# UBCMOCCA/mocca_envs

Measured on AMD Instinct MI355X. Metric: env-steps/sec, Walker3DCustomEnv-v0 @ 4096 envs, 1/2/4/8 MI355X, higher is better.
Workload: dtype f32; 1 GPU; Walker3DCustomEnv-v0, 4096 envs/GPU, flat ground, U(-1,1) action tape, auto-reset; max_rows=48, max_contacts=12, envs_per_gpu=4096, parallelism=independent env shards x1, no collective, preroll_steps=5896

## Files before the change

### mocca_envs_amd/csrc/mocca_device.h

```cpp
#pragma once

#include <hip/hip_runtime.h>
#include <stdint.h>

#include "mocca_model.h"
#include "mocca_philox.h"
#include "topo_walker3d.h"
#include "topo_cassie.h"
#include "topo_walker2d.h"
#include "topo_crab2d.h"
#include "topo_laikago.h"

#define DI __device__ __forceinline__

#ifndef MOCCA_NS
#define MOCCA_NS mocca
#endif
#ifndef MOCCA_MAXR
#define MOCCA_MAXR 48
#endif
#ifndef MOCCA_COMPACT
#define MOCCA_COMPACT 0
#endif

// ... 872 lines not shown
DI float hf_height_at(const float* hf, int rows, int cols, float sc, float x, float y) {
  const float ox = (float)rows / sc * 0.5f, oy = (float)cols / sc * 0.5f;
  int ix = (int)((x + ox) * sc), iy = (int)((y + oy) * sc);
  ix = ix < 0 ? 0 : (ix > cols - 1 ? cols - 1 : ix);
  iy = iy < 0 ? 0 : (iy > rows - 1 ? rows - 1 : iy);
  return hf[iy * cols + ix];
}

DI float clamp01(float x) { return x < 0.0f ? 0.0f : (x > 1.0f ? 1.0f : x); }
DI void seg_seg(const float* p1, const float* q1, const float* p2, const float* q2, float* c1, float* c2) {
  float d1[3], d2[3], r[3];
#pragma unroll
  for (int k = 0; k < 3; ++k) { d1[k] = q1[k] - p1[k]; d2[k] = q2[k] - p2[k]; r[k] = p1[k] - p2[k]; }
  const float a = dot3(d1, d1), e = dot3(d2, d2), f = dot3(d2, r), EPS = 1e-12f;
  float s, t;
  if (a <= EPS && e <= EPS) { s = t = 0; }
  else if (a <= EPS) { s = 0; t = clamp01(f * rcp(e)); }
  else {
    const float c = dot3(d1, r), ia = rcp(a);
    if (e <= EPS) { t = 0; s = clamp01(-c * ia); }
    else {
      const float b = dot3(d1, d2), den = a * e - b * b;
      s = den > EPS ? clamp01((b * f - c * e) * rcp(den)) : 0.0f;
      t = (b * s + f) * rcp(e);
      if (t < 0) { t = 0; s = clamp01(-c * ia); }
      else if (t > 1) { t = 1; s = clamp01((b - c) * ia); }
    }
  }
#pragma unroll
  for (int k = 0; k < 3; ++k) { c1[k] = p1[k] + d1[k] * s; c2[k] = p2[k] + d2[k] * t; }
}

template <class T>
DI void geom_points(ModelP M, float* L, int lane) {
  static_assert(6 * T::NG <= GP_FLOATS || (T::NPAIR == 0 && !COMPACT), "geom points would overlap the contact records read by the self-collision pass");
  if (lane < 2 * T::NG) {
    const f4_t t = *(CF4P)(M->gp_tab[lane]);
    const int b = __float_as_int(t.w);
    const float pl[3] = {t.x, t.y, t.z};
#pragma unroll
    for (int i = 0; i < 3; ++i) {
      const float4 fr = *reinterpret_cast<const float4*>(L + L_RT + 12 * b + 4 * i);
      L[L_GP + 3 * lane + i] = fr.x * pl[0] + fr.y * pl[1] + fr.z * pl[2] + fr.w;
    }
  }
}

DI void stage_planks(ModelP M, float* L, int lane, const float* ter) {
  if (lane < M->n_planks) {
    const int row = (int)ter[120 + lane];
    const float* ti = ter + 6 * row;
    float Rb[9];
    euler_to_mat(ti[4], ti[5], ti[3], Rb);
    const float cz = M->plank_com_z, dz = -M->plank_half[2] - cz;
#pragma unroll
    for (int i = 0; i < 9; ++i) L[L_PLANK + 12 * lane + i] = Rb[i];
    L[L_PLANK + 12 * lane + 9] = ti[0] + Rb[2] * dz;
    L[L_PLANK + 12 * lane + 10] = ti[1] + Rb[5] * dz;
    L[L_PLANK + 12 * lane + 11] = ti[2] + Rb[8] * dz + cz;
  }
  wsync();
}

struct HeightFieldArgs { const float* data; int rows, cols; float scale; };
struct ContactFlags { int touch0, touch1, target0, target1, touch2, touch3, body_touch, target2, target3; };
DI int cover_targets(int cover, int nsi, int n_planks, int f) { return (cover >> (4 * f + nsi % n_planks)) & 1; }

template <class T, int TASK>
DI ContactFlags collide(ModelP M, float* L, int lane, const float* ter, int next_step_index,
                        int* nc_out, int32_t* dbg, int* nc_wanted, const HeightFieldArgs hfa, int* cover_out = nullptr) {
  STAMP_BEGIN;
  const float mreach = unif(M->contact_margin);
  ContactFlags fl = {0, 0, 0, 0, 0, 0, 0, 0, 0};
  const int maxc = uni(M->max_contacts);
  bool active = false;
  float n[3] = {0, 0, 1}, P[3] = {0, 0, 0}, gap = 1e30f, mu = 0, erp = M->erp, cfm = 0;
  int body = -1, slot = lane, cover_k = -1 , gfoot = -1, gtorso = 0;
  unsigned bmask = 0u;
  if (lane < T::NSLOT) {
    const f4_t st = *(CF4P)(M->slot_tab[lane]);
    const int ids = __float_as_int(st.z);
    const int g = (ids >> 8) & 0xFF, e = (ids >> 16) & 1;
    bmask = __float_as_uint(st.w);
    if ((ids >> 25) & 1) {
      gfoot = ((ids >> 26) & 7) - 1;
      gtorso = (ids >> 29) & 1;
      float C[3], Cw[3];
      const float rad = st.x, gfric = st.y;
#pragma unroll
      for (int i = 0; i < 3; ++i) { C[i] = L[L_GP + 3 * (2 * g + e) + i]; Cw[i] = C[i] + L[L_BASE + i]; }
      body = ids & 0xFF;
      if (TASK == MOCCA_TASK_WALKER3D_PLANNER) {
        gap = sphere_heightfield(hfa.data, hfa.rows, hfa.cols, hfa.scale, Cw, rad, rad + mreach, 1 + ((ids >> 30) & 3), n);
        mu = M->plank_friction * gfric;
        const float kk = M->plank_stiffness, cc = M->plank_damping, dt = M->dt;
        const float ikc = rcp(dt * kk + cc);
        erp = dt * kk * ikc;
        cfm = ikc * rcp(dt);
      } else if (TASK != MOCCA_TASK_WALKER3D_STEPPER) {
        gap = Cw[2] - rad;
        mu = M->ground_friction * gfric;
      } else {
        const float h[3] = {M->plank_half[0], M->plank_half[1], M->plank_half[2]};
        const int n_planks = M->n_planks;
        const bool cyl = M->plank_shape == MOCCA_PLANK_CYLINDER;
#pragma unroll 1
        for (int k = 0; k < n_planks; ++k) {
          float Rb[9], bc[3], nn[3];
#pragma unroll
          for (int i = 0; i < 9; ++i) Rb[i] = L[L_PLANK + 12 * k + i];
#pragma unroll
          for (int i = 0; i < 3; ++i) bc[i] = L[L_PLANK + 12 * k + 9 + i];
          float lb[3];
// ... 67 lines not shown
      fl.target1 = cover_targets(cover, next_step_index, npl, 1);
      if constexpr (T::NFEET > 2) { fl.target2 = cover_targets(cover, next_step_index, npl, 2); fl.target3 = cover_targets(cover, next_step_index, npl, 3); }
      if (cover_out) *cover_out = cover;
    }
    if (TASK == MOCCA_TASK_WALKER3D_PLANNER) fl.body_touch = __ballot(active && gtorso) != 0ull;
  }
  int nc = __popcll(am);
  const int n_terrain = nc;
  int n_self = 0;
  unsigned long long kept = am;
  if (nc > maxc) {
    int deeper = 0;
    for (unsigned long long mm = am; mm; mm &= mm - 1) {
      const int l = __builtin_ctzll(mm);
      const float gl = readlane(gap, l);
      deeper += (gl < gap || (gl == gap && l < lane)) ? 1 : 0;
    }
    kept = __ballot(active && deeper < maxc);
  }
  {
    const int idx = lane_rank(kept);
    if (active && ((kept >> lane) & 1ull)) {
      float* ct = L + L_CT + 16 * idx;
      ct[C_BA] = __int_as_float(body); ct[C_BB] = __int_as_float(-1); ct[C_SLOT] = __int_as_float(slot);
#pragma unroll
      for (int i = 0; i < 3; ++i) { ct[C_P + i] = P[i]; ct[C_N + i] = n[i]; }
      ct[C_DEPTH] = -gap; ct[C_MU] = mu; ct[C_ERP] = erp; ct[C_CFM] = cfm;
      ct[C_MA] = __uint_as_float(bmask); ct[C_MB] = __uint_as_float(0u);
    }
  }
  if (nc > maxc) nc = maxc;
  STAMP(13);
  const int npairs = uni(M->n_pairs);
  unsigned short* cand = reinterpret_cast<unsigned short*>(L + L_CAND);
  static_assert(2 * ((COMPACT ? L_ABA_END : L_TOTAL) - L_CAND) >= MOCCA_MAX_PAIRS, "candidate list must hold every pair");
  int ncand = 0;
#pragma unroll 1
  for (int base = 0; base < npairs; base += 64) {
    const int k = base + lane;
    bool near = false;
    if (k < npairs) {
#ifdef MOCCA_ABL_PAIRLOAD
      f4_t pt;
      pt.x = __int_as_float((k % T::NG) | (((k * 7 + 3) % T::NG) << 5) | (24 << 20)); pt.y = 0.05f; pt.z = 0.05f; pt.w = 0.04f;
#else
      const f4_t pt = *(CF4P)(M->pair_tab[k]);
#endif
      const int ids = __float_as_int(pt.x);
      const int ga = ids & 31, gb = (ids >> 5) & 31;
      float dm[3];
#pragma unroll
      for (int i = 0; i < 3; ++i)
        dm[i] = (L[L_GP + 6 * ga + i] + L[L_GP + 6 * ga + 3 + i]) - (L[L_GP + 6 * gb + i] + L[L_GP + 6 * gb + 3 + i]);
      const float reach = 2.0f * (pt.w + (float)((ids >> 20) & 0xFF) * (1.0f / 8192.0f));
      near = dot3(dm, dm) < reach * reach;
    }
    const unsigned long long nm = __ballot(near);
    if (near) cand[ncand + lane_rank(nm)] = (unsigned short)k;
    ncand += __popcll(nm);
  }
  ncand = uni(ncand);
#ifdef MOCCA_ABL_NOPASS2
  ncand = 0;
#endif
  wsync();
#pragma unroll 1
  for (int base = 0; base < ncand; base += 64) {
    bool hit = false;
    float nn[3] = {0, 0, 0}, PP[3] = {0, 0, 0}, g2 = 0, mu2 = 0;
    int ba = -1, bb = -1;
    if (base + lane < ncand) {
      const int k = cand[base + lane];
      const f4_t pt = *(CF4P)(M->pair_tab[k]);
      const int ids = __float_as_int(pt.x);
      const int ga = ids & 31, gb = (ids >> 5) & 31;
      float a1[3], a2[3], b1[3], b2[3];
#pragma unroll
      for (int i = 0; i < 3; ++i) {
        a1[i] = L[L_GP + 6 * ga + i]; a2[i] = L[L_GP + 6 * ga + 3 + i];
// ... 194 lines not shown
#pragma unroll 1
  for (int j = nnc - 1; j >= 0; --j) {
    const float as = Acol[MAXR * j] * invdiag;
    const float nl_ = __builtin_amdgcn_fmed3f(y, lo0, 1e30f);
    const float dl = readlane(nl_ - lam, j);
    lam = lane == j ? nl_ : lam;
    y = fmaf(-as, dl, y);
  }
}
template <int PGS_REG_ROWS, int RR>
DI void pgs_fixed_rows_from(const float* Acol, const float* ar, int start, int r_fr, float& y, float& lam, float invdiag, float lo0) {
  if constexpr (RR < MAXR) {
    if (RR >= r_fr) return;
    if (RR >= start) pgs_visit<RR>(RR < PGS_REG_ROWS ? ar[RR < PGS_REG_ROWS ? RR : 0] : Acol[MAXR * RR] * invdiag, y, lam, lo0);
    pgs_fixed_rows_from<PGS_REG_ROWS, RR + 1>(Acol, ar, start, r_fr, y, lam, invdiag, lo0);
  }
}

DI void set_issue_priority(int nr, int prio) {
  if (nr > ((prio >> 12) & 63)) __builtin_amdgcn_s_setprio(3);
  else if (nr > ((prio >> 6) & 63)) __builtin_amdgcn_s_setprio(2);
  else if (nr > (prio & 63)) __builtin_amdgcn_s_setprio(1);
  else __builtin_amdgcn_s_setprio(0);
}
#ifndef MOCCA_PACE_ROWUNIT
#define MOCCA_PACE_ROWUNIT 2
#endif
#ifndef MOCCA_PACE_SHIFT
#define MOCCA_PACE_SHIFT 4
#endif
constexpr int PACE_TICK_SHIFT = 6;
enum : int { L_T0 = L_BASE + 13, L_PACE = L_BASE + 14, L_KEEPWARM = L_BASE + 15  };
constexpr unsigned PACE_CNT_BITS = 24, PACE_WINDOW = 128;
DI void pace_start(const StepArgs& a, float* L, int lane, int pace) {
  if (lane == 0) {
    int p16 = pace >> PACE_TICK_SHIFT;
    if (pace < 0) {
      const unsigned long long v = __hip_atomic_load(a.pace_acc, __ATOMIC_RELAXED, __HIP_MEMORY_SCOPE_AGENT);
      const unsigned cnt = (unsigned)v & ((1u << PACE_CNT_BITS) - 1u);
      p16 = cnt > 0u ? (int)((float)(v >> PACE_CNT_BITS) / (float)cnt * (float)(-pace) * 0.0625f) : 0;
    }
    L[L_PACE] = __int_as_float(p16);
    if (pace != 0) L[L_T0] = __uint_as_float((unsigned)__builtin_amdgcn_s_memtime());
  }
}
DI void pace_finish(const StepArgs& a, const float* L, int lane, int pace) {
  if (pace < 0 && lane == 0 && (blockIdx.x % 61u) == 0u) {
    const unsigned el = ((unsigned)__builtin_amdgcn_s_memtime() - __float_as_uint(L[L_T0])) >> PACE_TICK_SHIFT;
    const unsigned long long old = atomicAdd(a.pace_acc, ((unsigned long long)el << PACE_CNT_BITS) | 1ull);
    if (((unsigned)old & ((1u << PACE_CNT_BITS) - 1u)) + 1u == PACE_WINDOW) {
      const unsigned long long sum = (old >> PACE_CNT_BITS) + el;
      atomicAdd(a.pace_acc, 0ull - (((sum >> 1) << PACE_CNT_BITS) | (unsigned long long)(PACE_WINDOW / 2)));
    }
  }
}
DI bool pace_on(const float* L) { return uni(__float_as_int(L[L_PACE])) > 0; }
DI void pace_checkpoint(const float* L, int done, int total) {
  const unsigned p16 = (unsigned)uni(__float_as_int(L[L_PACE]));
  if (p16 == 0u) return;
  const unsigned el = (unsigned)__builtin_amdgcn_s_memtime() - (unsigned)uni(__float_as_int(L[L_T0]));
  const unsigned lhs = (el >> PACE_TICK_SHIFT) * (unsigned)total, r = p16 * (unsigned)done;
  if (lhs > r + (r >> MOCCA_PACE_SHIFT)) __builtin_amdgcn_s_setprio(3);
  else if (lhs > r) __builtin_amdgcn_s_setprio(2);
  else if (lhs > r - (r >> MOCCA_PACE_SHIFT)) __builtin_amdgcn_s_setprio(1);
  else __builtin_amdgcn_s_setprio(0);
}
DI void dbg_fold_step(int32_t* dbg, int lane) {
  if (dbg && lane == 0) {
    unsigned long long h = ((unsigned long long)(unsigned)dbg[17] << 32) | (unsigned)dbg[16];
#pragma unroll 1
    for (int w = 0; w < 12; ++w) h = (h ^ (unsigned long long)(unsigned)dbg[w]) * 0x9E3779B97F4A7C15ull;
    dbg[16] = (int32_t)(unsigned)h; dbg[17] = (int32_t)(unsigned)(h >> 32); dbg[18] += 1;
  }
}
template <class T>
DI void solve_constraints(ModelP M, float* L, int lane, int nc_found, int nc_wanted, unsigned long long ppk, int32_t* dbg, const float* Afac, int prio, int& rows_out) {
  const bool keep_warm = uni(__float_as_int(L[L_KEEPWARM])) != 0;
  STAMP_BEGIN;
  const float dt = unif(M->dt), idt = rcp(dt);
  const int maxr = uni(M->max_rows);
  int nl;
  {
    bool act = false;
    if (lane < 2 * T::NJ) {
      const int b = 1 + (lane >> 1), side = lane & 1;
      const float q = L[L_Q + b];
      const float gap = side == 0 ? q - M->jlo[b] : M->jhi[b] - q;
      const float vel = (side == 0 ? 1.0f : -1.0f) * L[L_NU + 5 + b];
      act = M->limit_at_violation ? !(gap > 0.0f) : gap + dt * vel < M->limit_slack;
    }
    const unsigned long long lm = __ballot(act);
    const int rk = lane_rank(lm);
    if (act && rk < maxr) reinterpret_cast<int*>(L)[L_ROWD + rk] = lane;
    nl = uni(__popcll(lm));
    if (dbg && lane == 0) {
      dbg[5] = (int32_t)(unsigned)lm; dbg[6] = (int32_t)(unsigned)(lm >> 32);
      const int nfix = 3 * T::NCLOS + ((T::NCLOS > 0 && M->planar) ? 3 : 0), mc = M->max_contacts;
      const int wanted = nl + nfix + 3 * nc_wanted;
      dbg[12] += nc_wanted > mc ? 1 : 0;
      dbg[13] += nl + nfix + 3 * (nc_wanted < mc ? nc_wanted : mc) > maxr ? 1 : 0;
      dbg[14] += 1;
      if (wanted > dbg[15]) dbg[15] = wanted;
    }
    if (nl > maxr) nl = maxr;
  }
  constexpr int NCL = 3 * T::NCLOS;
  const int NFIX = NCL + ((T::NCLOS > 0 && uni(M->planar)) ? 3 : 0);
  int nc = uni(nc_found);
  if (nc > (maxr - nl - NFIX) / 3) nc = (maxr - nl - NFIX) / 3;
  if (nc < 0) nc = 0;
  const int nr = nl + NFIX + 3 * nc;
  if (dbg && lane == 0) { dbg[0] = nr; dbg[1] = nl; dbg[2] = nc; }
  if (!pace_on(L)) set_issue_priority(nr, prio);
  rows_out = nr;
  wsync();
  STAMP(16);
  if (nr == 0) {
    if (dbg && lane == 0) { dbg[8] = 0; dbg[9] = 0; dbg[10] = 0; dbg[11] = 0; }
    if (keep_warm && lane < T::NSLOT) L[L_WARM + lane] = 0.0f;
    wsync();
    return;
  }
  const int r = lane;
  const int r_fr = nl + NFIX + nc;
  const int row_gap = MAXR - nr;
  const bool is_fric = r >= MAXR - 2 * nc && r < MAXR;
  const bool has_row = r < r_fr || is_fric;
  const int ci = is_fric ? (MAXR - 1 - r) >> 1 : r - nl - NFIX;
  int kind = -1, ba = 0, bb = -1, jl = -1, slot = -1;
  float F[6] = {0, 0, 0, 0, 0, 0}, sgn = 0, bias = 0, cfm = 0, lam = 0, mu = 0;
  float F2[6] = {0, 0, 0, 0, 0, 0};
  if (r < nl) {
    const int c = reinterpret_cast<int*>(L)[L_ROWD + r];
    const int b = 1 + (c >> 1), side = c & 1;
    const float q = L[L_Q + b];
    const float gap = side == 0 ? q - M->jlo[b] : M->jhi[b] - q;
    kind = 0; jl = b; ba = b; sgn = side == 0 ? 1.0f : -1.0f;
    bias = gap < 0 ? M->erp_noncontact * (-gap) * idt : -gap * idt;
  } else if (T::NCLOS > 0 && r < nl + NCL) {
    const int c = (r - nl) / 3, ax = (r - nl) % 3;
    ba = M->cl_body_a[c]; bb = M->cl_body_b[c];
    kind = 3;
    float Pa[3], Pb[3], Ra[9], Rb[9], la[3], lb[3];
#pragma unroll
    for (int x = 0; x < 9; ++x) { Ra[x] = L[L_RT + 12 * ba + 4 * (x / 3) + x % 3]; Rb[x] = L[L_RT + 12 * bb + 4 * (x / 3) + x % 3]; }
#pragma unroll
    for (int x = 0; x < 3; ++x) { la[x] = M->cl_point_a[c][x]; lb[x] = M->cl_point_b[c][x]; }
    matvec3(Ra, la, Pa); matvec3(Rb, lb, Pb);
#pragma unroll
    for (int x = 0; x < 3; ++x) { Pa[x] += L[L_RT + 12 * ba + 4 * x + 3]; Pb[x] += L[L_RT + 12 * bb + 4 * x + 3]; }
    float dir[3] = {ax == 0 ? 1.0f : 0.0f, ax == 1 ? 1.0f : 0.0f, ax == 2 ? 1.0f : 0.0f}, pn[3];
    cross3(Pa, dir, pn);
#pragma unroll
    for (int x = 0; x < 3; ++x) { F[x] = pn[x]; F[3 + x] = dir[x]; }
    cross3(Pb, dir, pn);
#pragma unroll
    for (int x = 0; x < 3; ++x) { F2[x] = pn[x]; F2[3 + x] = dir[x]; }
    const float e = ax == 0 ? Pb[0] - Pa[0] : (ax == 1 ? Pb[1] - Pa[1] : Pb[2] - Pa[2]);
    bias = M->erp_noncontact * e * idt;
  } else if (T::NCLOS > 0 && r < nl + NFIX) {
    const int k = r - nl - NCL;
    const int comp = k == 0 ? 0 : (k == 1 ? 2 : 4);
    kind = 3; ba = 0; bb = -1;
#pragma unroll
    for (int x = 0; x < 6; ++x) F[x] = x == comp ? 1.0f : 0.0f;
    const float err = k == 0 ? L[L_RT + 9]  : (k == 1 ? -L[L_RT + 1]  : L[L_BASE + 1] - M->init_pos[1]);
    bias = -M->erp_noncontact * err * idt;
  } else if (has_row) {
    const float* ct = L + L_CT + 16 * ci;
    float n[3] = {ct[C_N], ct[C_N + 1], ct[C_N + 2]}, P[3] = {ct[C_P], ct[C_P + 1], ct[C_P + 2]}, dir[3];
    ba = __float_as_int(ct[C_BA]); bb = __float_as_int(ct[C_BB]);
    if (!is_fric) {
      kind = 1;
      dir[0] = n[0]; dir[1] = n[1]; dir[2] = n[2];
      const float depth = ct[C_DEPTH] - unif(M->linear_slop);
      bias = depth > 0 ? ct[C_ERP] * depth * idt : depth * idt;
      cfm = ct[C_CFM];
      slot = __float_as_int(ct[C_SLOT]);
      const float wsf = unif(M->warmstart);
      lam = (wsf != 0.0f && slot >= 0) ? wsf * L[L_WARM + slot] : 0.0f;
    } else {
      kind = 2;
      float t1[3], t2[3];
      plane_space(n, t1, t2);
      const bool second = (r & 1) != 0;
#pragma unroll
      for (int x = 0; x < 3; ++x) dir[x] = second ? t2[x] : t1[x];
      mu = ct[C_MU];
    }
    float pn[3];
    cross3(P, dir, pn);
#pragma unroll
    for (int x = 0; x < 3; ++x) { F[x] = pn[x]; F[3 + x] = dir[x]; F2[x] = pn[x]; F2[3 + x] = dir[x]; }
  }
  STAMP(17);
  unsigned ma = 0u, mb = 0u;
  if (kind == 1 || kind == 2) {
    const float* ct = L + L_CT + 16 * ci;
    ma = __float_as_uint(ct[C_MA]); mb = __float_as_uint(ct[C_MB]);
  } else if (kind >= 0) {
    ma = M->anc_mask[ba];
    mb = (kind == 3 && bb >= 0) ? M->anc_mask[bb] : 0u;
  }
  const float sa = kind >= 1 ? 1.0f : 0.0f, sb = (kind >= 1 && bb >= 0) ? 1.0f : 0.0f;

  STAMP(5);
  float X[T::ND];
  float w = 0;
  const int dense = has_row ? (r < r_fr ? r : r - row_gap) : MAXR;
  float* Jrow = L + L_J + 28 * dense;
  float pa[6] = {0, 0, 0, 0, 0, 0}, pb[6] = {0, 0, 0, 0, 0, 0};
#ifdef MOCCA_NO_TWO_PATHS
  const bool two_paths = false;
#else
  const bool two_paths = T::NCLOS > 0 || __ballot(kind >= 1 && bb >= 0) != 0ull;
#endif
  STAMP(18);
  const unsigned long long pka = ((unsigned long long)(unsigned)__shfl((int)(unsigned)(ppk >> 32), ba, 64) << 32) |
                                 (unsigned long long)(unsigned)__shfl((int)(unsigned)ppk, ba, 64);
  {
    float4* jz = reinterpret_cast<float4*>(Jrow);
#pragma unroll
    for (int i = 1; i < 7; ++i) jz[i] = make_float4(0.0f, 0.0f, 0.0f, 0.0f);
  }
  float pu[T::MAXD], pub[T::MAXD];
#pragma unroll
  for (int k = T::MAXD - 1; k >= 0; --k) {
    const int j = (int)((pka >> (5 * k)) & 31ull);
    const bool valid = j != 0;
    const int jj = j;
    float S[6], U[6];
#pragma unroll
    for (int i = 0; i < 6; ++i) { S[i] = L[L_SV + SVS * jj + i]; U[i] = L[L_SV + SVS * jj + SV_V + i]; }
    float jb = dot6(S, F);
    if (jj == jl) jb = sgn;
// ... 248 lines not shown
    float ax[3], jr[9], Rq[9], Tl[9];
#pragma unroll
    for (int i = 0; i < 3; ++i) ax[i] = M->jaxis[j][i];
#pragma unroll
    for (int i = 0; i < 9; ++i) jr[i] = M->jrot[j][i];
    Rq[0] = cq + t * ax[0] * ax[0];          Rq[1] = t * ax[0] * ax[1] - s * ax[2];   Rq[2] = t * ax[0] * ax[2] + s * ax[1];
    Rq[3] = t * ax[0] * ax[1] + s * ax[2];   Rq[4] = cq + t * ax[1] * ax[1];          Rq[5] = t * ax[1] * ax[2] - s * ax[0];
    Rq[6] = t * ax[0] * ax[2] - s * ax[1];   Rq[7] = t * ax[1] * ax[2] + s * ax[0];   Rq[8] = cq + t * ax[2] * ax[2];
    matmul3(jr, Rq, Tl);
    float4* rec = reinterpret_cast<float4*>(L + L_SV + SVS * j);
    rec[0] = make_float4(Tl[0], Tl[1], Tl[2], Tl[3]);
    rec[1] = make_float4(Tl[4], Tl[5], Tl[6], Tl[7]);
    rec[2] = make_float4(Tl[8], M->jpos[j][0], M->jpos[j][1], M->jpos[j][2]);
    rec[3] = make_float4(ax[0], ax[1], ax[2], L[L_QD + j]);
  }
  wsync();
}

template <class T, int TASK>
DI ContactFlags substep(ModelP M, float* L, int lane, const float* ter, int next_step_index,
                        unsigned long long ppk, int32_t* dbg, int prio, int& rows_out,
                        const HeightFieldArgs hfa = HeightFieldArgs{nullptr, 0, 0, 0.0f}, int sidx = 0, int nsub = 1, int* cover_out = nullptr) {
  const int per0 = 64 + MOCCA_PACE_ROWUNIT * rows_out, done0 = sidx * per0, total = nsub * per0;
  STAMP(30);
  stage_joints<T>(M, L, lane);
  STAMP(29);
  int nc = 0, nc_wanted = 0;
  float Afac[21] = {0, 0, 0, 0, 0, 0, 0, 0, 0, 0, 0, 0, 0, 0, 0, 0, 0, 0, 0, 0, 0};
  ContactFlags fl = {0, 0, 0, 0, 0, 0, 0, 0, 0};
  if constexpr (COMPACT) {
    static_assert(!COMPACT || T::NCLOS == 0, "closure rows read the body frames after the ABA: not in the compact layout");
    int wl = lane;
    asm volatile("" : "+v"(wl));
    walk_phase1<T>(L, wl, ppk);
    wsync();
    STAMP(0);
    geom_points<T>(M, L, lane);
    wsync();
    STAMP(15);
#ifndef MOCCA_SKIP_COLLIDE
    fl = collide<T, TASK>(M, L, lane, ter, next_step_index, &nc, dbg, &nc_wanted, hfa, cover_out);
#endif
    wsync();
    const int wb = wl < T::NB ? wl : 0;
    WalkConsts wk;
    walk_consts<true>(M, wb, wk);
    walk_phase2<T, true>(M, L, wl, wb, ppk, wk);
    wsync();
  } else {
    walk_kinematics<T, true>(M, L, lane, ppk);
    wsync();
    STAMP(0);
    geom_points<T>(M, L, lane);
    wsync();
    STAMP(15);
#ifndef MOCCA_SKIP_COLLIDE
    fl = collide<T, TASK>(M, L, lane, ter, next_step_index, &nc, dbg, &nc_wanted, hfa, cover_out);
#endif
  }
  STAMP(1);
  pace_checkpoint(L, done0 + 20, total);
#ifndef MOCCA_SKIP_ABA
  aba_passes<T>(M, L, lane, ppk, Afac);
#endif
  STAMP(2);
  pace_checkpoint(L, done0 + 36, total);
#ifndef MOCCA_SKIP_SOLVE
  solve_constraints<T>(M, L, lane, nc, nc_wanted, ppk, dbg, Afac, prio, rows_out);
#endif
  if (dbg) { __builtin_amdgcn_s_waitcnt(0); dbg_fold_step(dbg, lane); }
  STAMP(3);
#ifdef MOCCA_DUMMY_VALU
  {
    float x = (float)lane;
#ifdef MOCCA_DUMMY_ILP
    float y = x + 1.0f, z = x + 2.0f, u = x + 3.0f;
#pragma unroll 1
    for (int i = 0; i < MOCCA_DUMMY_VALU; ++i) { x = fmaf(x, 1.0001f, 0.5f); y = fmaf(y, 0.9999f, -0.5f); z = fmaf(z, 1.0001f, 0.5f); u = fmaf(u, 0.9999f, -0.5f); }
    asm volatile("" :: "v"(y), "v"(z), "v"(u));
#else
#pragma unroll 1
    for (int i = 0; i < MOCCA_DUMMY_VALU; ++i) { x = fmaf(x, 1.0001f, 0.5f); x = fmaf(x, 0.9999f, -0.5f); x = fmaf(x, 1.0001f, 0.5f); x = fmaf(x, 0.9999f, -0.5f); }
#endif
    asm volatile("" :: "v"(x));
  }
#endif
  integrate<T>(M, L, lane);
  STAMP(4);
  pace_checkpoint(L, (sidx + 1) * (64 + MOCCA_PACE_ROWUNIT * rows_out), nsub * (64 + MOCCA_PACE_ROWUNIT * rows_out));
  return fl;
// ... 429 lines not shown
  if (mode != MOCCA_CASSIE_PLAIN) {
    const float u = draw_u<INJECT>(a, env, t.episode, t.draw);
    t.draw += 1;
    int is = (int)(u * 10000.0f);
    is = is > 9999 ? 9999 : is;
    t.istep = M->cassie_rsi ? is : 0;
    frame = traj_frame(a, M, t.istep, &phase);
  }
  if (lane >= 1 && lane < T::NB) { L[L_Q + lane] = M->init_q[lane]; L[L_QD + lane] = 0.0f; }
  if (lane < MOCCA_MAX_CTRL) L[L_JVEL + lane] = 0.0f;
  wsync();
  if (mode != MOCCA_CASSIE_PLAIN) {
    const float* fr = a.traj + (size_t)frame * MOCCA_TRAJ_STRIDE;
    if (lane < M->n_ordered) {
      const int b = M->ordered_body[lane];
      L[L_Q + b] = fr[lane]; L[L_QD + b] = fr[14 + lane]; L[L_JVEL + lane] = fr[14 + lane];
    }
    if (lane < 4) { L[L_Q + M->rod_body[lane]] = fr[28 + lane]; L[L_QD + M->rod_body[lane]] = 0.0f; }
  }
  t.initz = reset_base_pose<T>(M, L, lane);
  const CassieState cs = cassie_state(M, L, lane, t.initz);
  cassie_observe(M, L, lane, cs, t.initz, lane < MOCCA_MAX_CTRL ? L[L_JVEL + lane] : 0.0f, phase, obs);
  t.linpot = cassie_potential(M, L);
}

template <class T, int TASK, bool INJECT>
DI void reset_task(const StepArgs& a, ModelP M, float* L, float* ter, uint32_t* tk, int env, int lane, TaskRegs& t, float* obs) {
  if constexpr (TASK == MOCCA_TASK_CASSIE) {
    cassie_reset_env<T, INJECT>(a, M, L, env, lane, t, obs);
    if (lane < MOCCA_MAX_CTRL) tk[MOCCA_TW_JVEL + lane] = __float_as_uint(L[L_JVEL + lane]);
  } else reset_env<T, TASK, INJECT>(a, M, L, ter, env, lane, t, obs);
}

DI void load_dyn(const float* st, float* L, int lane, int nj, int nslots, bool warm = true) {
  if (lane < 13) L[L_BASE + lane] = st[lane];
  if (lane < nj) { L[L_Q + 1 + lane] = st[13 + lane]; L[L_QD + 1 + lane] = st[13 + nj + lane]; }
  if (warm) { if (lane < nslots) L[L_WARM + lane] = st[13 + 2 * nj + lane]; }
  else if (lane < MOCCA_MAX_SLOTS) L[L_WARM + lane] = 0.0f;
}
DI void store_dyn(float* st, const float* L, int lane, int nj, int nslots, bool warm = true) {
  if (lane < 13) st[lane] = L[L_BASE + lane];
  if (lane < nj) { st[13 + lane] = L[L_Q + 1 + lane]; st[13 + nj + lane] = L[L_QD + 1 + lane]; }
  if (warm && lane < nslots) st[13 + 2 * nj + lane] = L[L_WARM + lane];
}

}
```

### mocca_envs_amd/csrc/mocca_kernels.h

```cpp
#pragma once
#include <hip/hip_runtime.h>

#include "mocca.h"
#include "mocca_device.h"

namespace MOCCA_NS {

#ifndef MOCCA_WAVES_PER_EU
#define MOCCA_WAVES_PER_EU 4
#endif

DI void flush_obs(const float* L, float* dst, int lane, int obs_dim) {
#pragma unroll 1
  for (int k = lane; k < obs_dim; k += 64) dst[k] = L[L_OBS + k];
}
DI void keep_terminal_obs(const StepArgs& a, const float* L, int env, int lane) {
  wsync();
  if (a.final_obs) flush_obs(L, a.final_obs + (size_t)env * a.obs_dim, lane, a.obs_dim);
  wsync();
}

template <class T>
DI void keep_robot_state(const StepArgs& a, const float* L, int env, int lane) {
  static_assert(ROBOT_OBS<T> <= 64 && ROBOT_OBS<T> <= ROBOT_STATE_STRIDE, "one store per lane");
// ... 179 lines not shown
template <class T>
DI StepResult cassie_step(const StepArgs& __restrict__ a, ModelP M, float* L, uint32_t* tk, int lane, unsigned long long ppk, TaskRegs& __restrict__ t,
                          float* obs) {
  t.istep += M->n_llc;
  float jv = 0.0f;
  if (lane < M->n_ordered) {
    jv = (L[L_Q + M->ordered_body[lane]] - L[L_Q0 + lane]) / M->control_dt;
    tk[MOCCA_TW_JVEL + lane] = __float_as_uint(jv);
  }
  stage_joints<T>(M, L, lane);
  walk_kinematics<T, false>(M, L, lane, ppk);
  wsync();
  t.t += 1;
  const CassieState cs = cassie_state(M, L, lane, t.initz);
  const float old = t.linpot;
  t.linpot = cassie_potential(M, L);
  const float alive = cs.height > M->alive_height ? 2.0f : -1.0f;
  if (!cs.finite || alive < 0.0f) t.done = 1;
  float rew = alive + (t.linpot - old);
  float phase = 0.0f;
  if (M->cassie_mode != MOCCA_CASSIE_PLAIN) {
    const int f1 = traj_frame(a, M, t.istep, &phase);
    rew = cassie_mocap_reward(a, M, L, lane, cs, jv, f1);
  }
  cassie_observe(M, L, lane, cs, t.initz, jv, phase, obs);
  return {rew, 0};
}

template <class T, int TASK, bool INJECT = false>
__global__ __launch_bounds__(64, MOCCA_WAVES_PER_EU) void mocca_step_kernel(StepArgs a) {
  __shared__ float L[L_TOTAL];
  const int lane = threadIdx.x;
  if ((int)blockIdx.x >= a.n_envs) return;
  const int env = a.order ? uni(a.order[blockIdx.x]) : (int)blockIdx.x;
  ModelP M = (ModelP)a.model;
  float* st = a.dyn + (size_t)env * DYN_STRIDE;
  uint32_t* tk = a.task + (size_t)env * MOCCA_TASK_WORDS;
  float* ter = TASK == MOCCA_TASK_WALKER3D_STEPPER ? a.terrain + (size_t)env * TERRAIN_STRIDE : nullptr;
  float* obs_out = a.obs + (size_t)env * a.obs_dim;
  float* obs = L + L_OBS;
  int32_t* dbg = a.dbg ? a.dbg + (size_t)env * MOCCA_DEBUG_WORDS : nullptr;

  const bool warm_ld = INJECT || uni(__float_as_int(M->warmstart)) != 0, warm_st = warm_ld || a.persist_warm != 0;
  if (dbg && lane == 0) { dbg[16] = 0; dbg[17] = 0; dbg[18] = 0; }
  load_dyn(st, L, lane, T::NJ, T::NSLOT, warm_ld);
  pace_start(a, L, lane, INJECT ? 0 : a.pace);
  if (lane == 0) L[L_KEEPWARM] = __int_as_float(warm_st ? 1 : 0);
  const unsigned long long ppk = T::path_packed(lane < T::NB ? lane : 0);
  ContactFlags fl = {0, 0, 0, 0, 0, 0, 0, 0, 0};
  int cover = 0;
  if constexpr (TASK == MOCCA_TASK_CASSIE) {
    const int no = M->n_ordered, nctl = M->n_ctrl, mode = M->cassie_mode;
    float target = 0.0f;
    if (lane < nctl) {
      float base = M->ctrl_base[lane];
      if (mode != MOCCA_CASSIE_PLAIN) {
        const int f0 = traj_frame(a, M, (int)tk[MOCCA_TW_ISTEP]);
        base = (lane < nctl - 2 && M->residual_control) ? a.traj[(size_t)f0 * MOCCA_TRAJ_STRIDE + M->ctrl_oidx[lane]] : 0.0f;
      }
      target = base + (lane < nctl - 2 ? a.act[(size_t)env * (nctl - 2) + lane] : 0.0f);
    }
    if (lane < no) {
      L[L_JVEL + lane] = __uint_as_float(tk[MOCCA_TW_JVEL + lane]);
      L[L_Q0 + lane] = L[L_Q + M->ordered_body[lane]];
    }
    if (lane < MOCCA_MAX_BODIES) L[L_TAU + lane] = 0.0f;
    if (lane == 0) { L[L_Q] = 0.0f; L[L_QD] = 0.0f; }
    wsync();
    const int nllc = INJECT ? 0 : M->n_llc;
    int last_rows = uni((int)tk[MOCCA_TW_LAST_ROWS]);
    if (!INJECT && a.pace == 0) set_issue_priority(last_rows, a.prio);
#pragma unroll 1
    for (int it = 0; it < nllc; ++it) {
      ModelP Ms = M;
      int ln = lane;
      unsigned long long pk = ppk;
      asm volatile("" : "+s"(Ms), "+v"(ln), "+v"(pk));
      if (ln < no) {
        const float al = Ms->jvel_alpha;
        L[L_JVEL + ln] = (1.0f - al) * L[L_JVEL + ln] + al * L[L_QD + Ms->ordered_body[ln]];
      }
      wsync();
      if (ln < nctl) {
        const int b = Ms->ctrl_body[ln];
        const float perr = target - L[L_Q + b];
        float verr = -L[L_JVEL + Ms->ctrl_oidx[ln]];
        verr = verr < -5.0f ? -5.0f : (verr > 5.0f ? 5.0f : verr);
        const float tq = Ms->ctrl_kp[ln] * perr + Ms->ctrl_kd[ln] * verr, lim = Ms->torque_limit[b];
        L[L_TAU + b] = tq < -lim ? -lim : (tq > lim ? lim : tq);
      }
      wsync();
      substep<T, TASK>(Ms, L, ln, nullptr, 0, pk, dbg, a.prio, last_rows, HeightFieldArgs{nullptr, 0, 0, 0.0f}, it, nllc);
    }
    if (!INJECT && lane == 0) tk[MOCCA_TW_LAST_ROWS] = (uint32_t)last_rows;
  } else {
    {
      const float applied_gain = __uint_as_float(tk[MOCCA_TW_APPLIED_GAIN]);
      if (lane < T::NJ) {
        const float act_raw = a.act[(size_t)env * T::NJ + lane];
        const float c = act_raw < -1.0f ? -1.0f : (act_raw > 1.0f ? 1.0f : act_raw);
        L[L_TAU + 1 + lane] = M->gain[lane + 1] * applied_gain * c;
      }
    }
    if (lane == 0) { L[L_TAU] = 0.0f; L[L_Q] = 0.0f; L[L_QD] = 0.0f; }
    wsync();

    STAMP(28);
    if constexpr (TASK == MOCCA_TASK_WALKER3D_STEPPER) stage_planks(M, L, lane, ter);
    const int nsub = INJECT ? 0 : M->n_substeps;
    const int nsi0 = TASK == MOCCA_TASK_WALKER3D_STEPPER ? (int)tk[MOCCA_TW_NEXT_STEP_INDEX] : 0;
    int last_rows = uni((int)tk[MOCCA_TW_LAST_ROWS]);
    if (!INJECT && a.pace == 0) set_issue_priority(last_rows, a.prio);
#pragma unroll 1
    for (int s = 0; s < nsub; ++s) {
      ModelP Ms = M;
      int ln = lane;
      unsigned long long pk = ppk;
      asm volatile("" : "+s"(Ms), "+v"(ln), "+v"(pk));
      fl = substep<T, TASK>(Ms, L, ln, ter, nsi0, pk, dbg, a.prio, last_rows, HeightFieldArgs{a.hf, a.hf_rows, a.hf_cols, a.hf_scale}, s, nsub, &cover);
    }
    if constexpr (INJECT) {
      const int32_t* tc = a.inj_touch + (size_t)env * T::NFEET;
      fl.touch0 = tc[0] != 0; fl.touch1 = tc[1] != 0;
      if constexpr (T::NFEET > 2) { fl.touch2 = tc[2] != 0; fl.touch3 = tc[3] != 0; }
      if (a.inj_target) {
        const int32_t* tg = a.inj_target + (size_t)env * T::NFEET;
        const int npl = TASK == MOCCA_TASK_WALKER3D_STEPPER ? M->n_planks : 1;
#pragma unroll
        for (int f = 0; f < T::NFEET; ++f)
          if (tg[f] == 1 || tg[f] == 2) cover |= 1 << (4 * f + (nsi0 + tg[f] - 1) % npl);
        fl.target0 = tg[0] == 1; fl.target1 = tg[1] == 1;
        if constexpr (T::NFEET > 2) { fl.target2 = tg[2] == 1; fl.target3 = tg[3] == 1; }
      }
      if (a.inj_body) fl.body_touch = a.inj_body[env] != 0;
    }
    if (!INJECT && lane == 0) tk[MOCCA_TW_LAST_ROWS] = (uint32_t)last_rows;
    STAMP(27);
  }
  TaskRegs t = load_task<T, TASK>(tk);
  const float ep_ret0 = a.ep_ret ? a.ep_ret[env] : 0.0f;
  StepResult r;
  if constexpr (TASK == MOCCA_TASK_CASSIE) r = cassie_step<T>(a, M, L, tk, lane, ppk, t, obs);
  else {
    const float act_raw = lane < T::NJ ? a.act[(size_t)env * T::NJ + lane] : 0.0f;
    {
      int lo = lane;
      asm volatile("" : "+v"(lo));
      stage_joints<T>(M, L, lo);
      walk_kinematics<T, false>(M, L, lo, ppk);
    }
    wsync();
    t.t += 1;
// ... 121 lines not shown
```

Baseline: 41.13 million env-steps/s.

## Issue global loads early and pin them in registers across kernel phases

```diff
diff --git a/mocca_envs_amd/csrc/mocca_device.h b/mocca_envs_amd/csrc/mocca_device.h
--- a/mocca_envs_amd/csrc/mocca_device.h
+++ b/mocca_envs_amd/csrc/mocca_device.h
@@ -928,10 +928,12 @@
 }
 
 template <class T>
-DI void geom_points(ModelP M, float* L, int lane) {
+DI f4_t geom_request(ModelP M, int lane) { return *(CF4P)(M->gp_tab[lane < 2 * T::NG ? lane : 0]); }
+template <class T>
+DI void geom_points(float* L, int lane, f4_t t) {
   static_assert(6 * T::NG <= GP_FLOATS || (T::NPAIR == 0 && !COMPACT), "geom points would overlap the contact records read by the self-collision pass");
+  asm volatile("" : "+v"(t));
   if (lane < 2 * T::NG) {
-    const f4_t t = *(CF4P)(M->gp_tab[lane]);
     const int b = __float_as_int(t.w);
     const float pl[3] = {t.x, t.y, t.z};
 #pragma unroll
@@ -958,13 +960,15 @@
   wsync();
 }
 
+template <class T>
+DI f4_t slot_request(ModelP M, int lane) { return *(CF4P)(M->slot_tab[lane < T::NSLOT ? lane : 0]); }
 struct HeightFieldArgs { const float* data; int rows, cols; float scale; };
 struct ContactFlags { int touch0, touch1, target0, target1, touch2, touch3, body_touch, target2, target3; };
 DI int cover_targets(int cover, int nsi, int n_planks, int f) { return (cover >> (4 * f + nsi % n_planks)) & 1; }
 
 template <class T, int TASK>
 DI ContactFlags collide(ModelP M, float* L, int lane, const float* ter, int next_step_index,
-                        int* nc_out, int32_t* dbg, int* nc_wanted, const HeightFieldArgs hfa, int* cover_out = nullptr) {
+                        int* nc_out, int32_t* dbg, int* nc_wanted, const HeightFieldArgs hfa, f4_t slot_rec, int* cover_out = nullptr) {
   STAMP_BEGIN;
   const float mreach = unif(M->contact_margin);
   ContactFlags fl = {0, 0, 0, 0, 0, 0, 0, 0, 0};
@@ -973,8 +977,9 @@
   float n[3] = {0, 0, 1}, P[3] = {0, 0, 0}, gap = 1e30f, mu = 0, erp = M->erp, cfm = 0;
   int body = -1, slot = lane, cover_k = -1 , gfoot = -1, gtorso = 0;
   unsigned bmask = 0u;
+  asm volatile("" : "+v"(slot_rec));
   if (lane < T::NSLOT) {
-    const f4_t st = *(CF4P)(M->slot_tab[lane]);
+    const f4_t st = slot_rec;
     const int ids = __float_as_int(st.z);
     const int g = (ids >> 8) & 0xFF, e = (ids >> 16) & 1;
     bmask = __float_as_uint(st.w);
@@ -1108,6 +1113,8 @@
   if (nc > maxc) nc = maxc;
   STAMP(13);
   const int npairs = uni(M->n_pairs);
+  f4_t pt_next = {0.0f, 0.0f, 0.0f, 0.0f};
+  if (npairs > 0) pt_next = *(CF4P)(M->pair_tab[lane < npairs ? lane : npairs - 1]);
   unsigned short* cand = reinterpret_cast<unsigned short*>(L + L_CAND);
   static_assert(2 * ((COMPACT ? L_ABA_END : L_TOTAL) - L_CAND) >= MOCCA_MAX_PAIRS, "candidate list must hold every pair");
   int ncand = 0;
@@ -1115,12 +1122,15 @@
   for (int base = 0; base < npairs; base += 64) {
     const int k = base + lane;
     bool near = false;
+    f4_t pt_cur = pt_next;
+    if (base + 64 < npairs) pt_next = *(CF4P)(M->pair_tab[k + 64 < npairs ? k + 64 : npairs - 1]);
+    asm volatile("" : "+v"(pt_cur));
     if (k < npairs) {
 #ifdef MOCCA_ABL_PAIRLOAD
       f4_t pt;
       pt.x = __int_as_float((k % T::NG) | (((k * 7 + 3) % T::NG) << 5) | (24 << 20)); pt.y = 0.05f; pt.z = 0.05f; pt.w = 0.04f;
 #else
-      const f4_t pt = *(CF4P)(M->pair_tab[k]);
+      const f4_t pt = pt_cur;
 #endif
       const int ids = __float_as_int(pt.x);
       const int ga = ids & 31, gb = (ids >> 5) & 31;
@@ -1381,11 +1391,13 @@
 constexpr int PACE_TICK_SHIFT = 6;
 enum : int { L_T0 = L_BASE + 13, L_PACE = L_BASE + 14, L_KEEPWARM = L_BASE + 15  };
 constexpr unsigned PACE_CNT_BITS = 24, PACE_WINDOW = 128;
-DI void pace_start(const StepArgs& a, float* L, int lane, int pace) {
+DI unsigned long long pace_request(const StepArgs& a, int pace) {
+  return pace < 0 ? __hip_atomic_load(a.pace_acc, __ATOMIC_RELAXED, __HIP_MEMORY_SCOPE_AGENT) : 0ull;
+}
+DI void pace_start(const StepArgs& a, float* L, int lane, int pace, unsigned long long v) {
   if (lane == 0) {
     int p16 = pace >> PACE_TICK_SHIFT;
     if (pace < 0) {
-      const unsigned long long v = __hip_atomic_load(a.pace_acc, __ATOMIC_RELAXED, __HIP_MEMORY_SCOPE_AGENT);
       const unsigned cnt = (unsigned)v & ((1u << PACE_CNT_BITS) - 1u);
       p16 = cnt > 0u ? (int)((float)(v >> PACE_CNT_BITS) / (float)cnt * (float)(-pace) * 0.0625f) : 0;
     }
@@ -1426,17 +1438,25 @@
 DI void solve_constraints(ModelP M, float* L, int lane, int nc_found, int nc_wanted, unsigned long long ppk, int32_t* dbg, const float* Afac, int prio, int& rows_out) {
   const bool keep_warm = uni(__float_as_int(L[L_KEEPWARM])) != 0;
   STAMP_BEGIN;
+  const int bl = lane < 2 * T::NJ ? 1 + (lane >> 1) : 1;
+  float jlo_l = M->jlo[bl], jhi_l = M->jhi[bl];
+  unsigned anc_l = M->anc_mask[bl];
   const float dt = unif(M->dt), idt = rcp(dt);
   const int maxr = uni(M->max_rows);
+  const int lim_viol = M->limit_at_violation;
+  const float lim_slack = M->limit_slack;
+  float gap_l = 0.0f;
+  asm volatile("" : "+v"(jlo_l), "+v"(jhi_l), "+v"(anc_l));
   int nl;
   {
     bool act = false;
     if (lane < 2 * T::NJ) {
-      const int b = 1 + (lane >> 1), side = lane & 1;
+      const int b = bl, side = lane & 1;
       const float q = L[L_Q + b];
-      const float gap = side == 0 ? q - M->jlo[b] : M->jhi[b] - q;
+      const float gap = side == 0 ? q - jlo_l : jhi_l - q;
       const float vel = (side == 0 ? 1.0f : -1.0f) * L[L_NU + 5 + b];
-      act = M->limit_at_violation ? !(gap > 0.0f) : gap + dt * vel < M->limit_slack;
+      act = lim_viol ? !(gap > 0.0f) : gap + dt * vel < lim_slack;
+      gap_l = gap;
     }
     const unsigned long long lm = __ballot(act);
     const int rk = lane_rank(lm);
@@ -1479,11 +1499,13 @@
   int kind = -1, ba = 0, bb = -1, jl = -1, slot = -1;
   float F[6] = {0, 0, 0, 0, 0, 0}, sgn = 0, bias = 0, cfm = 0, lam = 0, mu = 0;
   float F2[6] = {0, 0, 0, 0, 0, 0};
+  const int rc = reinterpret_cast<int*>(L)[L_ROWD + (r < nl ? r : 0)];
+  const float gap_r = __shfl(gap_l, rc, 64);
+  const unsigned anc_r = (unsigned)__shfl((int)anc_l, rc, 64);
   if (r < nl) {
-    const int c = reinterpret_cast<int*>(L)[L_ROWD + r];
+    const int c = rc;
     const int b = 1 + (c >> 1), side = c & 1;
-    const float q = L[L_Q + b];
-    const float gap = side == 0 ? q - M->jlo[b] : M->jhi[b] - q;
+    const float gap = gap_r;
     kind = 0; jl = b; ba = b; sgn = side == 0 ? 1.0f : -1.0f;
     bias = gap < 0 ? M->erp_noncontact * (-gap) * idt : -gap * idt;
   } else if (T::NCLOS > 0 && r < nl + NCL) {
@@ -1547,9 +1569,11 @@
   if (kind == 1 || kind == 2) {
     const float* ct = L + L_CT + 16 * ci;
     ma = __float_as_uint(ct[C_MA]); mb = __float_as_uint(ct[C_MB]);
-  } else if (kind >= 0) {
+  } else if (kind == 0) {
+    ma = anc_r;
+  } else if (T::NCLOS > 0 && kind == 3) {
     ma = M->anc_mask[ba];
-    mb = (kind == 3 && bb >= 0) ? M->anc_mask[bb] : 0u;
+    mb = bb >= 0 ? M->anc_mask[bb] : 0u;
   }
   const float sa = kind >= 1 ? 1.0f : 0.0f, sb = (kind >= 1 && bb >= 0) ? 1.0f : 0.0f;
 
@@ -1864,14 +1888,16 @@
     static_assert(!COMPACT || T::NCLOS == 0, "closure rows read the body frames after the ABA: not in the compact layout");
     int wl = lane;
     asm volatile("" : "+v"(wl));
+    const f4_t gq = geom_request<T>(M, lane);
     walk_phase1<T>(L, wl, ppk);
     wsync();
     STAMP(0);
-    geom_points<T>(M, L, lane);
+    const f4_t sq = slot_request<T>(M, lane);
+    geom_points<T>(L, lane, gq);
     wsync();
     STAMP(15);
 #ifndef MOCCA_SKIP_COLLIDE
-    fl = collide<T, TASK>(M, L, lane, ter, next_step_index, &nc, dbg, &nc_wanted, hfa, cover_out);
+    fl = collide<T, TASK>(M, L, lane, ter, next_step_index, &nc, dbg, &nc_wanted, hfa, sq, cover_out);
 #endif
     wsync();
     const int wb = wl < T::NB ? wl : 0;
@@ -1880,14 +1906,16 @@
     walk_phase2<T, true>(M, L, wl, wb, ppk, wk);
     wsync();
   } else {
+    const f4_t gq = geom_request<T>(M, lane);
     walk_kinematics<T, true>(M, L, lane, ppk);
     wsync();
     STAMP(0);
-    geom_points<T>(M, L, lane);
+    const f4_t sq = slot_request<T>(M, lane);
+    geom_points<T>(L, lane, gq);
     wsync();
     STAMP(15);
 #ifndef MOCCA_SKIP_COLLIDE
-    fl = collide<T, TASK>(M, L, lane, ter, next_step_index, &nc, dbg, &nc_wanted, hfa, cover_out);
+    fl = collide<T, TASK>(M, L, lane, ter, next_step_index, &nc, dbg, &nc_wanted, hfa, sq, cover_out);
 #endif
   }
   STAMP(1);
@@ -2383,11 +2411,28 @@
   } else reset_env<T, TASK, INJECT>(a, M, L, ter, env, lane, t, obs);
 }
 
+struct DynRegs { float base, q, qd, warm; };
+DI DynRegs dyn_request(const float* st, int lane, int nj, int nslots, bool warm = true) {
+  DynRegs d;
+  d.base = st[lane < 13 ? lane : 12];
+  const int lj = lane < nj ? lane : nj - 1;
+  d.q = st[13 + lj];
+  d.qd = st[13 + nj + lj];
+  d.warm = 0.0f;
+  if (warm) d.warm = st[13 + 2 * nj + (lane < nslots ? lane : nslots - 1)];
+  return d;
+}
+DI void dyn_pin(DynRegs& d) { asm volatile("" : "+v"(d.base), "+v"(d.q), "+v"(d.qd), "+v"(d.warm)); }
+DI void dyn_commit(const DynRegs& d, float* L, int lane, int nj, int nslots, bool warm = true) {
+  if (lane < 13) L[L_BASE + lane] = d.base;
+  if (lane < nj) { L[L_Q + 1 + lane] = d.q; L[L_QD + 1 + lane] = d.qd; }
+  if (warm) { if (lane < nslots) L[L_WARM + lane] = d.warm; }
+  else if (lane < MOCCA_MAX_SLOTS) L[L_WARM + lane] = 0.0f;
+}
 DI void load_dyn(const float* st, float* L, int lane, int nj, int nslots, bool warm = true) {
-  if (lane < 13) L[L_BASE + lane] = st[lane];
-  if (lane < nj) { L[L_Q + 1 + lane] = st[13 + lane]; L[L_QD + 1 + lane] = st[13 + nj + lane]; }
-  if (warm) { if (lane < nslots) L[L_WARM + lane] = st[13 + 2 * nj + lane]; }
-  else if (lane < MOCCA_MAX_SLOTS) L[L_WARM + lane] = 0.0f;
+  DynRegs d = dyn_request(st, lane, nj, nslots, warm);
+  dyn_pin(d);
+  dyn_commit(d, L, lane, nj, nslots, warm);
 }
 DI void store_dyn(float* st, const float* L, int lane, int nj, int nslots, bool warm = true) {
   if (lane < 13) st[lane] = L[L_BASE + lane];
diff --git a/mocca_envs_amd/csrc/mocca_kernels.h b/mocca_envs_amd/csrc/mocca_kernels.h
--- a/mocca_envs_amd/csrc/mocca_kernels.h
+++ b/mocca_envs_amd/csrc/mocca_kernels.h
@@ -235,6 +235,7 @@
   __shared__ float L[L_TOTAL];
   const int lane = threadIdx.x;
   if ((int)blockIdx.x >= a.n_envs) return;
+  STAMP(31);
   const int env = a.order ? uni(a.order[blockIdx.x]) : (int)blockIdx.x;
   ModelP M = (ModelP)a.model;
   float* st = a.dyn + (size_t)env * DYN_STRIDE;
@@ -246,10 +247,22 @@
 
   const bool warm_ld = INJECT || uni(__float_as_int(M->warmstart)) != 0, warm_st = warm_ld || a.persist_warm != 0;
   if (dbg && lane == 0) { dbg[16] = 0; dbg[17] = 0; dbg[18] = 0; }
-  load_dyn(st, L, lane, T::NJ, T::NSLOT, warm_ld);
-  pace_start(a, L, lane, INJECT ? 0 : a.pace);
+  DynRegs dl = dyn_request(st, lane, T::NJ, T::NSLOT, warm_ld);
+  unsigned long long pacc = pace_request(a, INJECT ? 0 : a.pace);
+  unsigned long long ppk = T::path_packed(lane < T::NB ? lane : 0);
+  uint32_t w_rows = tk[MOCCA_TW_LAST_ROWS], w_gain = 0u, w_nsi = 0u;
+  float act_in = 0.0f, jgain = 0.0f;
+  if constexpr (TASK != MOCCA_TASK_CASSIE) {
+    const int lj = lane < T::NJ ? lane : T::NJ - 1;
+    w_gain = tk[MOCCA_TW_APPLIED_GAIN];
+    act_in = a.act[(size_t)env * T::NJ + lj];
+    jgain = M->gain[lj + 1];
+    if constexpr (TASK == MOCCA_TASK_WALKER3D_STEPPER) w_nsi = tk[MOCCA_TW_NEXT_STEP_INDEX];
+  }
+  asm volatile("" : "+v"(dl.base), "+v"(dl.q), "+v"(dl.qd), "+v"(dl.warm), "+v"(pacc), "+v"(ppk), "+v"(w_rows), "+v"(w_gain), "+v"(w_nsi), "+v"(act_in), "+v"(jgain));
+  dyn_commit(dl, L, lane, T::NJ, T::NSLOT, warm_ld);
+  pace_start(a, L, lane, INJECT ? 0 : a.pace, pacc);
   if (lane == 0) L[L_KEEPWARM] = __int_as_float(warm_st ? 1 : 0);
-  const unsigned long long ppk = T::path_packed(lane < T::NB ? lane : 0);
   ContactFlags fl = {0, 0, 0, 0, 0, 0, 0, 0, 0};
   int cover = 0;
   if constexpr (TASK == MOCCA_TASK_CASSIE) {
@@ -271,7 +284,7 @@
     if (lane == 0) { L[L_Q] = 0.0f; L[L_QD] = 0.0f; }
     wsync();
     const int nllc = INJECT ? 0 : M->n_llc;
-    int last_rows = uni((int)tk[MOCCA_TW_LAST_ROWS]);
+    int last_rows = uni((int)w_rows);
     if (!INJECT && a.pace == 0) set_issue_priority(last_rows, a.prio);
 #pragma unroll 1
     for (int it = 0; it < nllc; ++it) {
@@ -297,13 +310,9 @@
     }
     if (!INJECT && lane == 0) tk[MOCCA_TW_LAST_ROWS] = (uint32_t)last_rows;
   } else {
-    {
-      const float applied_gain = __uint_as_float(tk[MOCCA_TW_APPLIED_GAIN]);
-      if (lane < T::NJ) {
-        const float act_raw = a.act[(size_t)env * T::NJ + lane];
-        const float c = act_raw < -1.0f ? -1.0f : (act_raw > 1.0f ? 1.0f : act_raw);
-        L[L_TAU + 1 + lane] = M->gain[lane + 1] * applied_gain * c;
-      }
+    if (lane < T::NJ) {
+      const float c = act_in < -1.0f ? -1.0f : (act_in > 1.0f ? 1.0f : act_in);
+      L[L_TAU + 1 + lane] = jgain * __uint_as_float(w_gain) * c;
     }
     if (lane == 0) { L[L_TAU] = 0.0f; L[L_Q] = 0.0f; L[L_QD] = 0.0f; }
     wsync();
@@ -311,8 +320,8 @@
     STAMP(28);
     if constexpr (TASK == MOCCA_TASK_WALKER3D_STEPPER) stage_planks(M, L, lane, ter);
     const int nsub = INJECT ? 0 : M->n_substeps;
-    const int nsi0 = TASK == MOCCA_TASK_WALKER3D_STEPPER ? (int)tk[MOCCA_TW_NEXT_STEP_INDEX] : 0;
-    int last_rows = uni((int)tk[MOCCA_TW_LAST_ROWS]);
+    const int nsi0 = TASK == MOCCA_TASK_WALKER3D_STEPPER ? uni((int)w_nsi) : 0;
+    int last_rows = uni((int)w_rows);
     if (!INJECT && a.pace == 0) set_issue_priority(last_rows, a.prio);
 #pragma unroll 1
     for (int s = 0; s < nsub; ++s) {
@@ -320,7 +329,9 @@
       int ln = lane;
       unsigned long long pk = ppk;
       asm volatile("" : "+s"(Ms), "+v"(ln), "+v"(pk));
-      fl = substep<T, TASK>(Ms, L, ln, ter, nsi0, pk, dbg, a.prio, last_rows, HeightFieldArgs{a.hf, a.hf_rows, a.hf_cols, a.hf_scale}, s, nsub, &cover);
+      int hf_rows = a.hf_rows, hf_cols = a.hf_cols;
+      asm volatile("" : "+s"(hf_rows), "+s"(hf_cols));
+      fl = substep<T, TASK>(Ms, L, ln, ter, nsi0, pk, dbg, a.prio, last_rows, HeightFieldArgs{a.hf, hf_rows, hf_cols, a.hf_scale}, s, nsub, &cover);
     }
     if constexpr (INJECT) {
       const int32_t* tc = a.inj_touch + (size_t)env * T::NFEET;
```

Measured after the change: 41.44 million env-steps/s (median of 6 runs). Within noise of the previous version (+0.8%).
